# jiahuei/COMIC-Compact-Image-Captioning-with-Attention

Measured on AMD Instinct MI355X. Metric: images/sec (decoder-mode XE training, COMIC-256, InceptionV3 frozen), higher is better.
Workload: dtype bf16

## Files before the change

### comic-compact-image-captioning-with-attention_amd/_lib.py

```python
import ctypes as C
import os

_HERE = os.path.dirname(os.path.abspath(__file__))
LIB_PATH = os.environ.get('COMIC_HIP_LIB') or os.path.join(_HERE, 'lib', 'libcomic_hip.so')

c_void_p, c_int, c_int32, c_int64, c_float, c_double, c_char_p, c_uint64 = (
    C.c_void_p, C.c_int, C.c_int32, C.c_int64, C.c_float, C.c_double, C.c_char_p, C.c_uint64)


class CnnOp(C.Structure):
    _fields_ = [(n, c_int32) for n in (
        'kind', 'src', 'dst', 'src_coff', 'dst_coff', 'H', 'W', 'Cin', 'Cout', 'KH', 'KW', 'SH', 'SW',
        'PT', 'PL', 'Ho', 'Wo', 'weight', 'relu', 'out_f32', 'src_f32', 'lane', 'tile', 'group', 'flags', 'min_lds')]


class ImageDesc(C.Structure):
    _fields_ = [('offset', C.c_int64), ('in_h', c_int32), ('in_w', c_int32), ('flip', c_int32), ('oy', c_int32),
                ('ox', c_int32), ('sy', C.c_float), ('sx', C.c_float)]


class ConvWeight(C.Structure):
    _fields_ = [('w', c_void_p), ('scale', c_void_p), ('shift', c_void_p), ('w_frag', c_void_p)]


# ... 67 lines not shown
class BeamRequired(C.Structure):
    _fields_ = [('n_words', c_int32), ('stride', c_int32)]


class BeamSampling(C.Structure):
    _fields_ = [('temperature', c_float), ('seed_dev', c_void_p)]


class BeamTruncation(C.Structure):
    _fields_ = [('top_k', c_int32), ('top_p', c_float)]


class GemmProb(C.Structure):
    _fields_ = [(n, c_void_p) for n in ('A', 'B', 'C', 'bias', 'mask')] + [(n, c_int32) for n in (
        'M', 'N', 'K', 'lda', 'ldb', 'ldc', 'ld_mask')] + [(n, c_float) for n in ('alpha', 'beta', 'keep')] + [
        ('type', c_int32), ('ones_a', c_int32)]


class ConvGrad(C.Structure):
    _fields_ = [('w_master', c_void_p), ('dw', c_void_p), ('dbeta', c_void_p), ('w_bwd', c_void_p),
                ('bwd_tile', c_int32), ('reserved', c_int32)]


P = c_void_p
_SIGS = {
    'comic_last_error': (c_char_p, []),
    'comic_abi_version': (c_int, []),
    'comic_device_count': (c_int, []),
    'comic_pack_conv_weights': (c_int, [P, P, c_int, c_int, c_int, c_int, c_int, P]),
    'comic_fold_bn': (c_int, [P, P, P, c_float, P, P, c_int, P]),
    'comic_cnn_forward': (c_int, [P, c_int, P, P, P, c_int, c_int, P]),
    'comic_cnn_group_args_bytes': (C.c_long, [P, c_int]),
    'comic_cnn_build_group_args': (c_int, [P, c_int, P, P, P, c_int, P]),
    'comic_cnn_forward_grouped': (c_int, [P, c_int, P, P, P, c_int, c_int, P, P]),
    'comic_clip_by_norm': (c_int, [P, P, P, c_int, c_float, c_float, c_float, P, P, P]),
    'comic_cnn_backward_scratch_bytes': (c_int64, [P, c_int, c_int, c_int, c_int]),
    'comic_cnn_backward': (c_int, [P, c_int, P, P, P, P, P, c_int, c_int, c_int, P, c_int64, P, P]),
    'comic_cnn_backward_sched': (c_int, [P, c_int, P, c_int, P, P, P, P, P, P, c_int, c_int, c_int, P, c_int64, P, P, P]),
    'comic_cnn_pack_bwd_filters': (c_int, [P, c_int, P, c_int, P]),
    'comic_cnn_pack_x3_weights': (c_int, [P, P, P, P, P, c_int, P]),
    'comic_cnn_refresh_weights': (c_int, [P, P, c_int64, P, P, P, P, c_int64, P]),
    'comic_cnn_refresh_weights_dtype': (c_int, [P, P, c_int64, P, P, P, P, c_int64, c_int, P]),
    'comic_cnn_pack_frag_weights': (c_int, [P, P, P, c_int, c_int64, P]),
    'comic_crc32c': (C.c_uint32, [P, C.c_size_t, C.c_uint32]),
    'comic_conv2d_bn_relu': (c_int, [P, P, c_int, P, c_int, P, c_int, c_int, P]),
    'comic_gemm_f32': (c_int, [P, P, P, P, c_int, c_int, c_int, c_int, c_int, c_int, c_int, c_int, c_float,
                               c_float, P]),
    'comic_gemm_f32_split3': (c_int, [P, P, P, P, c_int, c_int, c_int, c_int, c_int, c_int, c_int, c_int, c_float,
                                      c_float, P, c_int64, P]),
    'comic_gemm_f32_splitk': (c_int, [P, P, P, P, c_int, c_int, c_int, c_int, c_int, c_int, c_int, c_int, c_float,
                                      c_float, P, c_int64, P]),
    'comic_gemm_group_workspace': (c_int64, [P, c_int]),
    'comic_gemm_group': (c_int, [P, c_int, P, c_int64, P]),
    'comic_embed_fwd': (c_int, [P, P, P, c_int, c_int, c_int, P]),
    'comic_embed_bwd': (c_int, [P, P, P, c_int, c_int, c_int, P]),
    'comic_dropout_apply': (c_int, [P, P, c_float, P, c_int64, P]),
    'comic_dropout_mask': (c_int, [P, c_int64, c_float, c_uint64, c_uint64, P]),
    'comic_dropout_mask_dev': (c_int, [P, c_int64, c_float, P, c_uint64, P]),
    'comic_dropout_masks4_dev': (c_int, [P, P, P, P, P]),
    'comic_image_preprocess': (c_int, [P, P, c_int, P, c_int, c_int, c_int, P]),
    'comic_jpeg_pixels': (c_int, [P, P, c_int, c_int, c_int, c_int, P, P, P]),
    'comic_jpeg_preprocess': (c_int, [P, P, c_int, c_int, P, P, P, P, c_int, c_int, c_int, P]),
    'comic_jpeg_preprocess_packed': (c_int, [P, P, c_int, c_int, P, P, P, P, c_int, c_int, c_int, P]),
    'comic_weighted_sum_tb': (c_int, [P, P, c_int, c_int, P, P]),
    'comic_lstm_gates_fwd': (c_int, [P, P, P, P, P, P, P, P, c_float, P, c_int, P, P, c_int, c_int, P]),
    'comic_lstm_gates_bwd': (c_int, [P, P, P, P, P, c_float, P, c_int, P, P, P, c_int, c_int, P]),
    'comic_attn_step_fwd': (c_int, [P, P, P, P, P, P, P, P, P, c_float, P, P, P, P]),
    'comic_attn_step_bwd': (c_int, [P, P, P, P, P, P, P, P, P, P, c_float, P, P, P, P, P, P, P]),
    'comic_xent_fwd_bwd': (c_int, [P, P, P, P, P, P, P, P, c_int, c_int, c_int, P]),
    'comic_argmax_rows': (c_int, [P, P, c_int, c_int, P]),
    'comic_beam_step': (c_int, [P, P, P, P, P, P, P, c_int, c_int, c_int, c_int, P]),
    'comic_gather_rows': (c_int, [P, P, P, c_int, c_int, c_int, P]),
    'comic_gather_tree': (c_int, [P, P, P, P, c_int, c_int, c_int, c_int, P]),
    'comic_adam_tf': (c_int, [P, P, P, P, c_int64, c_float, c_float, c_float, c_float, c_float, c_float, P]),
    'comic_adam_tf_gated': (c_int, [P, P, P, P, c_int64, c_float, c_float, c_float, c_float, c_float, c_float, P, P]),
    'comic_momentum_tf_gated': (c_int, [P, P, P, c_int64, c_float, c_float, c_float, c_float, P, P]),
    'comic_debug_occupy_cus': (c_int, [c_int, c_int, P]),
    'comic_colsum': (c_int, [P, P, c_int, c_int, c_float, P]),
    'comic_ln_tanh_fwd': (c_int, [P, P, P, P, P, c_int, c_int, c_float, P]),
    'comic_ln_tanh_bwd_rows': (c_int, [P, P, P, P, P, c_int, c_int, P]),
    'comic_momentum_tf': (c_int, [P, P, P, c_int64, c_float, c_float, c_float, c_float, P]),
    'comic_axpy': (c_int, [P, P, c_float, c_int64, P]),
    'comic_decoder_train_workspace': (c_int64, [P, c_int, c_int]),
    'comic_decoder_train_path': (c_int, []),
    'comic_decoder_greedy_path': (c_int, []),
    'comic_decoder_beam_path': (c_int, []),
    'comic_beam_step_dense_workspace': (c_int64, [c_int, c_int, c_int, c_int]),
    'comic_beam_step_dense': (c_int, [c_void_p] * 9 + [c_int] * 5 + [c_void_p, c_int64, c_void_p]),
    'comic_gemm_f32_stream_workspace': (c_int64, [c_int, c_int, c_int]),
    'comic_gemm_f32_stream': (c_int, [c_void_p, c_void_p, c_void_p, c_void_p, c_int, c_int, c_int, c_void_p, c_int64, c_void_p]),
    'comic_decoder_infer_workspace': (c_int64, [P, c_int, c_int]),
    'comic_decoder_train_step': (c_int, [P, P, P, P, P, P, P, P, P, P, c_int, c_int, c_int, P, P, P, P, P, P, P,
                                         P, P, P, P, P, c_int64, P]),
    'comic_decoder_score_workspace': (c_int64, [P, c_int, c_int]),
    'comic_decoder_score': (c_int, [P, P, P, P, P, P, P, P, c_int, c_int, c_int, P, P, P, P, c_int64, P]),
    'comic_decoder_score_path': (c_int, []),
    'comic_decoder_greedy': (c_int, [P, P, P, P, c_int, c_int, P, P, P, P, P, c_int64, P]),
    'comic_decoder_sample': (c_int, [P, P, P, P, c_int, c_int, P, P, P, P, P, P, c_int64, P]),
    'comic_decoder_beam': (c_int, [P, P, P, P, c_int, c_int, c_int, P, P, P, P, P, P, P, P, c_int64, P]),
    'comic_beam_step_ensemble_workspace': (c_int64, [c_int, c_int, c_int, c_int]),
    'comic_beam_step_ensemble': (c_int, [P, P, c_int, P, P, P, P, P, P, c_int, c_int, c_int, c_int, c_float, P, c_int64, P]),
    'comic_beam_step_ensemble_path': (c_int, []),
    'comic_decoder_beam_ensemble_workspace': (c_int64, [P, c_int, c_int, c_int]),
    'comic_decoder_beam_ensemble': (c_int, [P, P, P, P, P, c_int, c_int, c_int, c_int, P, P, P, P, P, P, P, P, c_int64, P]),
    'comic_beam_bans': (c_int, [P, P, P, P, P, P, c_int, c_int, c_int, c_int, c_int, c_int, P, P]),
    'comic_beam_step_constrained': (c_int, [P, P, c_int, P, P, P, P, P, P, c_int, c_int, c_int, c_int, c_float, P, c_int, P,
# ... 166 lines not shown
```

### comic-compact-image-captioning-with-attention_amd/csrc/gemm_group.h

```cpp
#pragma once
#include "common.h"

constexpr int kGemmGroupMax = 20;
enum { COMIC_GG_TN = 0, COMIC_GG_NN = 1, COMIC_GG_NT = 2 };

struct ComicGemmProb {
  const float* A;
  const float* B;
  float* C;
  const float* bias;
  const float* mask;
  int M, N, K, lda, ldb, ldc, ld_mask;
  float alpha, beta;
  float keep;
  int type;
  int ones_a;
  int tiles_m, tiles_n, S, k_per_slice, wg_begin;
  int slab_tile0;
  int ticket0;
};

struct ComicGemmGroup {
  ComicGemmProb p[kGemmGroupMax];
  int n;
  float* slab;
  unsigned* tickets;
  int xcd_chunk;
};

int comic_gemm_group_plan(ComicGemmGroup& g, int target_items, int64_t* slab_bytes, int* n_tickets);
constexpr int kGemmGroupTargetItems = 640;
int comic_gemm_group_launch(const ComicGemmGroup& g, int n_wg, hipStream_t st);
```

### comic-compact-image-captioning-with-attention_amd/csrc/gemm_group.hip

```cpp
#include <algorithm>

#include "gemm_group.h"
#include "gemm_x3_dev.h"

namespace {

constexpr int GB = 128;
constexpr int kGemmGroupSlots = 512;
constexpr int kItemOverhead = 6;
constexpr int kSc1 = 16;
typedef __attribute__((ext_vector_type(4))) unsigned gg_u32x4_t;

__device__ __forceinline__ __amdgpu_buffer_rsrc_t gg_rsrc(const void* p, long bytes) {
  return __builtin_amdgcn_make_buffer_rsrc((void*)p, 0, (int)bytes, 0x00020000);
}
__device__ __forceinline__ float4 gg_load16_sc1(__amdgpu_buffer_rsrc_t r, unsigned off) {
  const gg_u32x4_t v = __builtin_amdgcn_raw_buffer_load_b128(r, (int)off, 0, kSc1);
  return make_float4(__uint_as_float(v.x), __uint_as_float(v.y), __uint_as_float(v.z), __uint_as_float(v.w));
}
__device__ __forceinline__ void gg_store16_sc1(__amdgpu_buffer_rsrc_t r, unsigned off, float4 v) {
  const gg_u32x4_t u = {__float_as_uint(v.x), __float_as_uint(v.y), __float_as_uint(v.z), __float_as_uint(v.w)};
  __builtin_amdgcn_raw_buffer_store_b128(u, r, (int)off, 0, kSc1);
}

constexpr int kGroupLds = 4 * (X3Tile<GB, true>::BYTES + X3Tile<GB, true>::BYTES);
static_assert(X3Tile<GB, true>::BYTES >= X3Tile<GB, false>::BYTES, "LDS of the k-contiguous form bounds the others");
constexpr int kGroupLdsPc = 2 * 2 * (X3TilePc<GB, false>::BYTES + X3TilePc<GB, false>::BYTES);
static_assert(X3TilePc<GB, false>::BYTES >= X3TilePc<GB, true>::BYTES, "LDS of the row-contiguous form bounds the others");

__device__ __forceinline__ void gg_emit(const ComicGemmProb& p, int m, int n, float4 a) {
  if (m >= p.M || n >= p.N) return;
  const int nv = min(4, p.N - n);
  float v[4] = {a.x * p.alpha, a.y * p.alpha, a.z * p.alpha, a.w * p.alpha};
  float* cp = p.C + (size_t)m * p.ldc + n;
#pragma unroll
  for (int q = 0; q < 4; ++q) {
    if (q >= nv) break;
    if (p.bias) v[q] += p.bias[n + q];
    if (p.mask) v[q] = (v[q] / p.keep) * p.mask[(size_t)m * p.ld_mask + n + q];
    if (p.beta != 0.f) v[q] += p.beta * cp[q];
  }
  if (nv == 4 && (p.ldc % 4 == 0) && (((uintptr_t)p.C & 15) == 0)) {
    *(float4*)cp = make_float4(v[0], v[1], v[2], v[3]);
  } else {
#pragma unroll
    for (int q = 0; q < 4; ++q)
      if (q < nv) cp[q] = v[q];
  }
}

template <bool PC>
__global__ __launch_bounds__(PC ? 512 : 256) void gemm_group_x3_kernel(ComicGemmGroup g) {
  constexpr int NT = PC ? 512 : 256;
  constexpr int LDS = PC ? kGroupLdsPc : kGroupLds;
  extern __shared__ __attribute__((aligned(16))) unsigned char smem[];
  int bid = blockIdx.x;
  if (g.xcd_chunk > 0 && bid < g.xcd_chunk * 8) bid = (bid & 7) * g.xcd_chunk + (bid >> 3);
  volatile unsigned* s_last = (volatile unsigned*)(smem + LDS - 16);
  int pi = 0;
#pragma unroll 1
  for (int i = 1; i < g.n; ++i)
    if (bid >= g.p[i].wg_begin) pi = i;
  const ComicGemmProb& p = g.p[pi];
  const int local = bid - p.wg_begin;
  const int S = p.S, ntiles = p.tiles_m * p.tiles_n;
  const int slice = local / ntiles, tl = local - slice * ntiles;
  constexpr int PW = 8;
  const int panel = tl / (p.tiles_m * PW), rem = tl - panel * p.tiles_m * PW;
  const int pw = min(PW, p.tiles_n - panel * PW);
  const int mt = rem / pw, nt = panel * PW + rem % pw;
  const int tile = mt * p.tiles_n + nt;
  const int m0 = mt * GB, n0 = nt * GB;
  const int kbeg = S > 1 ? slice * p.k_per_slice : 0;
  const int kend = S > 1 ? min(p.K, kbeg + p.k_per_slice) : p.K;
  const int tid = threadIdx.x, lane = tid & 63, wave = tid >> 6;
  const int wm = wave >> 1, wn = wave & 1;

  const long tile_id = (long)p.ticket0 + tile;
  const __amdgpu_buffer_rsrc_t sr = gg_rsrc(g.slab + ((long)p.slab_tile0 + (long)tile * S) * (GB * GB), (long)S * GB * GB * 4);
  const unsigned sbase = (unsigned)slice * (GB * GB * 4);
  if (p.ones_a) {
    constexpr int KG = NT / 32;
    float4* red = (float4*)smem;
    const int cg = tid & 31, kg = tid >> 5, n = n0 + 4 * cg;
    const bool vec = (p.ldb % 4 == 0) && (((uintptr_t)p.B & 15) == 0);
    float4 sm = make_float4(0.f, 0.f, 0.f, 0.f);
    if (n < p.N)
      for (int k = kbeg + kg; k < kend; k += KG) {
        const float4 v = load4(p.B + (size_t)k * p.ldb + n, p.N - n, vec);
        sm.x += v.x; sm.y += v.y; sm.z += v.z; sm.w += v.w;
      }
    red[kg * 32 + cg] = sm;
    __syncthreads();
    if (tid < 32) {
      float4 tot = red[cg];
#pragma unroll
      for (int k = 1; k < KG; ++k) {
        const float4 v = red[k * 32 + cg];
        tot.x += v.x; tot.y += v.y; tot.z += v.z; tot.w += v.w;
      }
      if (S == 1) gg_emit(p, 0, n, tot);
      else gg_store16_sc1(sr, sbase + (unsigned)cg * 16u, tot);
    }
    if (S == 1) return;
  } else {
    f32x4_t acc[4][4];
    if constexpr (PC) {
      if (p.type == COMIC_GG_TN) x3_mainloop_pc<false, false>(p.A, p.B, p.M, p.N, p.lda, p.ldb, m0, n0, kbeg, kend, smem, acc);
      else if (p.type == COMIC_GG_NN) x3_mainloop_pc<true, false>(p.A, p.B, p.M, p.N, p.lda, p.ldb, m0, n0, kbeg, kend, smem, acc);
      else x3_mainloop_pc<true, true>(p.A, p.B, p.M, p.N, p.lda, p.ldb, m0, n0, kbeg, kend, smem, acc);
    } else {
      if (p.type == COMIC_GG_TN)
        x3_mainloop<GB, false, false, GB>(p.A, p.B, p.M, p.N, p.lda, p.ldb, m0, n0, kbeg, kend, smem, acc);
      else if (p.type == COMIC_GG_NN)
        x3_mainloop<GB, true, false, GB>(p.A, p.B, p.M, p.N, p.lda, p.ldb, m0, n0, kbeg, kend, smem, acc);
      else
        x3_mainloop<GB, true, true, GB>(p.A, p.B, p.M, p.N, p.lda, p.ldb, m0, n0, kbeg, kend, smem, acc);
    }
    const bool owner = wave < 4;
    if (S == 1) {
      if (owner)
#pragma unroll
      for (int i = 0; i < 4; ++i)
#pragma unroll
        for (int j = 0; j < 4; ++j)
          gg_emit(p, m0 + wm * 64 + j * 16 + (lane & 15), n0 + wn * 64 + i * 16 + (lane >> 4) * 4,
                  make_float4(acc[i][j][0], acc[i][j][1], acc[i][j][2], acc[i][j][3]));
      return;
    }
    if (owner)
#pragma unroll
    for (int i = 0; i < 4; ++i)
#pragma unroll
      for (int j = 0; j < 4; ++j) {
        const int ml = wm * 64 + j * 16 + (lane & 15), nl = wn * 64 + i * 16 + (lane >> 4) * 4;
        gg_store16_sc1(sr, sbase + (unsigned)(ml * GB + nl) * 4u, make_float4(acc[i][j][0], acc[i][j][1], acc[i][j][2], acc[i][j][3]));
      }
  }
  asm volatile("s_waitcnt vmcnt(0)" ::: "memory");
  __syncthreads();
  if (tid == 0) {
    const unsigned t = __hip_atomic_fetch_add(g.tickets + tile_id, 1u, __ATOMIC_RELAXED, __HIP_MEMORY_SCOPE_AGENT);
    *s_last = (t == (unsigned)(S - 1)) ? 1u : 0u;
    if (t == (unsigned)(S - 1)) __hip_atomic_store(g.tickets + tile_id, 0u, __ATOMIC_RELAXED, __HIP_MEMORY_SCOPE_AGENT);
  }
  __syncthreads();
  if (!*s_last) return;
  const int n_chunks = p.ones_a ? 1 : (GB * GB / 4) / NT;
#pragma unroll 1
  for (int c = 0; c < n_chunks; c += 4) {
    float4 sum[4];
#pragma unroll
    for (int u = 0; u < 4; ++u) sum[u] = make_float4(0.f, 0.f, 0.f, 0.f);
#pragma unroll 1
    for (int s = 0; s < S; ++s) {
      float4 v[4];
#pragma unroll
      for (int u = 0; u < 4; ++u) v[u] = gg_load16_sc1(sr, (unsigned)s * (GB * GB * 4) + (unsigned)(tid + NT * (c + u)) * 16u);
#pragma unroll
      for (int u = 0; u < 4; ++u) {
        sum[u].x += v[u].x; sum[u].y += v[u].y; sum[u].z += v[u].z; sum[u].w += v[u].w;
      }
    }
// ... 16 lines not shown
    COMIC_REQUIRE(p.M > 0 && p.N > 0 && p.K > 0 && p.B && p.C && (p.A || p.ones_a), "gemm_group: bad problem %d", i);
    COMIC_REQUIRE(p.type >= COMIC_GG_TN && p.type <= COMIC_GG_NT, "gemm_group: bad type of problem %d", i);
    COMIC_REQUIRE(!p.ones_a || (p.type == COMIC_GG_TN && p.M == 1), "gemm_group: ones_a needs type TN and M = 1 (problem %d)", i);
    COMIC_REQUIRE(p.ldc >= p.N && (!p.mask || p.ld_mask >= p.N), "gemm_group: leading dimension of problem %d", i);
    if (!p.ones_a) COMIC_REQUIRE(p.lda >= (p.type == COMIC_GG_TN ? p.M : p.K), "gemm_group: lda of problem %d", i);
    COMIC_REQUIRE(p.ldb >= (p.type == COMIC_GG_NT ? p.K : p.N), "gemm_group: ldb of problem %d", i);
    p.tiles_m = cdiv(p.M, GB);
    p.tiles_n = cdiv(p.N, GB);
    cost += (long)cdiv(p.M, GB) * p.tiles_n * cdiv(p.K, 32);
  }
  auto split_of = [](int kt, long klen) { return (int)std::min<long>(16, std::max<long>(1, (kt + klen / 2) / klen)); };
  long klen = std::max<long>(8, cost / std::max(1, target_items));
  {
    long best = -1, best_klen = klen, kt_max = 8;
    for (int i = 0; i < g.n; ++i) kt_max = std::max<long>(kt_max, cdiv(g.p[i].K, 32));
    for (long kl = klen; kl <= kt_max; ++kl) {
      long items = 0, longest = 0;
      for (int i = 0; i < g.n; ++i) {
        const ComicGemmProb& p = g.p[i];
        const int kt = cdiv(p.K, 32), S = split_of(kt, kl);
        items += (long)p.tiles_m * p.tiles_n * S;
        if (!p.ones_a) longest = std::max<long>(longest, cdiv(kt, S));
      }
      const long est = cdiv64(items, kGemmGroupSlots) * (longest + kItemOverhead);
      if (best < 0 || est < best) {
        best = est;
        best_klen = kl;
      }
    }
    klen = best_klen;
  }
  int wg = 0, tickets = 0, slab_tiles = 0;
  for (int i = 0; i < g.n; ++i) {
    ComicGemmProb& p = g.p[i];
    const int nt = cdiv(p.M, GB) * p.tiles_n, kt = cdiv(p.K, 32);
    int S = split_of(kt, klen);
    p.k_per_slice = cdiv(kt, S) * 32;
    S = cdiv(p.K, p.k_per_slice);
    p.S = S;
    p.wg_begin = wg;
    p.slab_tile0 = slab_tiles;
    p.ticket0 = tickets;
    wg += nt * S;
    if (S > 1) {
      slab_tiles += nt * S;
      tickets += nt;
    }
  }
  if (slab_bytes) *slab_bytes = (int64_t)slab_tiles * GB * GB * 4;
  if (n_tickets) *n_tickets = tickets;
  return wg;
}

int comic_gemm_group_launch(const ComicGemmGroup& g_in, int n_wg, hipStream_t st) {
  ComicGemmGroup g = g_in;
  g.xcd_chunk = n_wg / 8;
  COMIC_REQUIRE(n_wg > 0, "gemm_group: empty launch");
  bool pc = n_wg <= 256;
  for (int i = 0; i < g.n && pc; ++i) {
    const ComicGemmProb& p = g.p[i];
    if (p.ones_a) continue;
    const bool a_kc = p.type != COMIC_GG_TN, b_kc = p.type == COMIC_GG_NT;
    pc = p.lda % 4 == 0 && p.ldb % 4 == 0 && ((uintptr_t)p.A & 15) == 0 && ((uintptr_t)p.B & 15) == 0 &&
         (!(a_kc || b_kc) || p.K % 4 == 0);
  }
  static PerDeviceOnce once, once_pc;
  bool& done = pc ? once_pc.slot() : once.slot();
  const int lds = pc ? kGroupLdsPc : kGroupLds;
  if (!done) {
    const void* fn = pc ? (const void*)gemm_group_x3_kernel<true> : (const void*)gemm_group_x3_kernel<false>;
    COMIC_REQUIRE(hipFuncSetAttribute(fn, hipFuncAttributeMaxDynamicSharedMemorySize, lds) == hipSuccess,
                  "gemm_group: cannot reserve %d bytes of LDS", lds);
    done = true;
  }
  if (pc) hipLaunchKernelGGL(gemm_group_x3_kernel<true>, dim3((unsigned)n_wg), dim3(512), lds, st, g);
  else hipLaunchKernelGGL(gemm_group_x3_kernel<false>, dim3((unsigned)n_wg), dim3(256), lds, st, g);
  COMIC_LAUNCH_CHECK("gemm_group");
  return 0;
}

namespace {
int gg_from_public(const comic_gemm_prob* probs, int n, ComicGemmGroup& g) {
  COMIC_REQUIRE(probs && n > 0 && n <= kGemmGroupMax, "gemm_group: 1..%d problems", kGemmGroupMax);
  g = ComicGemmGroup{};
  g.n = n;
  for (int i = 0; i < n; ++i) {
    const comic_gemm_prob& q = probs[i];
    ComicGemmProb& p = g.p[i];
    p.A = q.A; p.B = q.B; p.C = q.C; p.bias = q.bias; p.mask = q.mask;
    p.M = q.M; p.N = q.N; p.K = q.K; p.lda = q.lda; p.ldb = q.ldb; p.ldc = q.ldc; p.ld_mask = q.ld_mask;
    p.alpha = q.alpha; p.beta = q.beta; p.keep = q.keep; p.type = q.type; p.ones_a = q.ones_a;
  }
  return 0;
}
#define kPublicTarget kGemmGroupTargetItems
}

extern "C" int64_t comic_gemm_group_workspace(const comic_gemm_prob* probs, int n) {
  ComicGemmGroup g;
  if (gg_from_public(probs, n, g)) return -1;
  int64_t slab = 0;
  int nt = 0;
  if (comic_gemm_group_plan(g, kPublicTarget, &slab, &nt) < 0) return -1;
  return slab + 256 + (int64_t)nt * 4;
}

extern "C" int comic_gemm_group(const comic_gemm_prob* probs, int n, void* workspace, int64_t workspace_bytes, void* stream) {
  ComicGemmGroup g;
  if (int rc = gg_from_public(probs, n, g)) return rc;
  int64_t slab = 0;
  int nt = 0;
  const int wg = comic_gemm_group_plan(g, kPublicTarget, &slab, &nt);
  if (wg < 0) return 2;
  const int64_t slab_al = (slab + 255) / 256 * 256;
  COMIC_REQUIRE(nt == 0 || (workspace && workspace_bytes >= slab_al + (int64_t)nt * 4), "gemm_group: workspace too small");
  g.slab = (float*)workspace;
  g.tickets = nt ? (unsigned*)((char*)workspace + slab_al) : nullptr;
  if (nt) COMIC_REQUIRE(hipMemsetAsync(g.tickets, 0, (size_t)nt * 4, (hipStream_t)stream) == hipSuccess, "gemm_group: memset");
  return comic_gemm_group_launch(g, wg, (hipStream_t)stream);
}
```

### comic-compact-image-captioning-with-attention_amd/csrc/gemm_x3_dev.h

```cpp
#pragma once
#include <type_traits>

#include "common.h"

namespace {

__device__ __forceinline__ float4 load4(const float* __restrict__ p, int nvalid, bool vec_ok) {
  if (nvalid >= 4 && vec_ok) return *(const float4*)p;
  float4 r = make_float4(0.f, 0.f, 0.f, 0.f);
  if (nvalid > 0) r.x = p[0];
  if (nvalid > 1) r.y = p[1];
  if (nvalid > 2) r.z = p[2];
  if (nvalid > 3) r.w = p[3];
  return r;
}

__device__ __forceinline__ void split_bf16x2(float a, float b, uint32_t& hi, uint32_t& lo) {
  hi = pack_bf16x2(a, b);
  lo = pack_bf16x2(a - __uint_as_float(hi << 16), b - __uint_as_float(hi & 0xFFFF0000u));
}

template <int ROWS, bool KC>
struct X3Tile {
  static constexpr int ROWB = 80;
// ... 205 lines not shown
    }
#pragma unroll
    for (int j = 0; j < TM; ++j) {
      ah[j] = x3_frag<BM, A_KC>(Ah + P * ABYTES, wm * (BM / 2) + j * 16, lane);
      al[j] = x3_frag<BM, A_KC>(Al + P * ABYTES, wm * (BM / 2) + j * 16, lane);
    }
#pragma unroll
    for (int i = 0; i < TN; ++i)
#pragma unroll
      for (int j = 0; j < TM; ++j) {
        acc[i][j] = __builtin_amdgcn_mfma_f32_16x16x32_bf16(bl[i], ah[j], acc[i][j], 0, 0, 0);
        acc[i][j] = __builtin_amdgcn_mfma_f32_16x16x32_bf16(bh[i], al[j], acc[i][j], 0, 0, 0);
        acc[i][j] = __builtin_amdgcn_mfma_f32_16x16x32_bf16(bh[i], ah[j], acc[i][j], 0, 0, 0);
      }
    sa.mask(kbeg + (kt + 1) * BKx, tid, ar[P ^ 1]);
    sb.mask(kbeg + (kt + 1) * BKx, tid, br[P ^ 1]);
    x3_store_tile<BM, A_KC, ACH>(Ah + (P ^ 1) * ABYTES, Al + (P ^ 1) * ABYTES, tid, ar[P ^ 1]);
    x3_store_tile<BN, B_KC, BCH>(Bh + (P ^ 1) * BBYTES, Bl + (P ^ 1) * BBYTES, tid, br[P ^ 1]);
#ifdef COMIC_X3_SCHED
    __builtin_amdgcn_sched_group_barrier(0x020, ACH + BCH, 0);
    __builtin_amdgcn_sched_group_barrier(0x100, 64, 0);
#pragma unroll
    for (int r = 0; r < TM * TN; ++r) {
      __builtin_amdgcn_sched_group_barrier(0x008, 3, 0);
      __builtin_amdgcn_sched_group_barrier(0x002, 9, 0);
      __builtin_amdgcn_sched_group_barrier(0x200, 1, 0);
    }
#endif
    __syncthreads();
  };
  for (int kt = 0; kt < nk; kt += 2) {
    step(kt, std::integral_constant<int, 0>());
    step(kt + 1, std::integral_constant<int, 1>());
  }
}

template <int BM, bool A_KC, bool B_KC, int BN>
__device__ __forceinline__ void x3_mainloop(const float* __restrict__ A, const float* __restrict__ B, int M, int N, int lda,
                                            int ldb, int m0, int n0, int kbeg, int kend, unsigned char* smem,
                                            f32x4_t (&acc)[BN / 32][BM / 32]) {
  const bool a_vec = (lda % 4 == 0) && (((uintptr_t)A & 15) == 0) && (!A_KC || kend % 4 == 0);
  const bool b_vec = (ldb % 4 == 0) && (((uintptr_t)B & 15) == 0) && (!B_KC || kend % 4 == 0);
  if (a_vec && b_vec) x3_mainloop_v<BM, A_KC, B_KC, BN, true>(A, B, M, N, lda, ldb, m0, n0, kbeg, kend, smem, acc);
  else x3_mainloop_v<BM, A_KC, B_KC, BN, false>(A, B, M, N, lda, ldb, m0, n0, kbeg, kend, smem, acc);
}

template <int ROWS, bool KC>
struct X3TilePc {
  static constexpr int KSTR = 2 * ROWS + 32;
  static constexpr int BYTES = KC ? ROWS * 64 : 32 * KSTR;
};
__device__ __forceinline__ int x3_swz(int row) { return (0x6C >> (((row >> 2) & 3) * 2)) & 3; }

template <int ROWS, bool KC, int NCH>
__device__ __forceinline__ void x3pc_store_tile(unsigned char* hi_base, unsigned char* lo_base, int tid,
                                                const float4 (&in)[NCH]) {
  using T = X3TilePc<ROWS, KC>;
#pragma unroll
  for (int i = 0; i < NCH; ++i) {
    const int q = tid + 256 * i;
    uint32_t h0, l0, h1, l1;
    split_bf16x2(in[i].x, in[i].y, h0, l0);
    split_bf16x2(in[i].z, in[i].w, h1, l1);
    int off;
    if (KC) {
      const int row = q >> 3, c = q & 7;
      off = row * 64 + (((c & 3) ^ x3_swz(row)) * 2 + (c >> 2)) * 8;
    } else {
      constexpr int CPR = ROWS / 4;
      const int kk = q / CPR, row = (q % CPR) * 4;
      off = kk * T::KSTR + row * 2;
    }
    *(uint2*)(hi_base + off) = make_uint2(h0, h1);
    *(uint2*)(lo_base + off) = make_uint2(l0, l1);
  }
}
template <int ROWS, bool KC>
__device__ __forceinline__ bf16x8_t x3pc_frag(const unsigned char* base, int row16, int lane) {
  using T = X3TilePc<ROWS, KC>;
  if (KC) {
    const int row = row16 + (lane & 15);
    const uint4 v = *(const uint4*)(base + row * 64 + (((lane >> 4) ^ x3_swz(row)) * 16));
    return __builtin_bit_cast(bf16x8_t, v);
  } else {
    const int g = lane >> 4, q = (lane >> 2) & 3, pp = lane & 3;
    const unsigned char* p = base + (4 * g + q) * T::KSTR + (row16 + 4 * pp) * 2;
    const uint32_t a0 = (uint32_t)(uintptr_t)((__attribute__((address_space(3))) const unsigned char*)p);
    const x3_s16x4_t lo = __builtin_amdgcn_ds_read_tr16_b64_v4i16((__attribute__((address_space(3))) x3_s16x4_t*)(uintptr_t)a0);
    const x3_s16x4_t hi =
        __builtin_amdgcn_ds_read_tr16_b64_v4i16((__attribute__((address_space(3))) x3_s16x4_t*)(uintptr_t)(a0 + 16 * T::KSTR));
    const x3_s16x8_t v = {lo[0], lo[1], lo[2], lo[3], hi[0], hi[1], hi[2], hi[3]};
    return __builtin_bit_cast(bf16x8_t, v);
  }
}

template <bool A_KC, bool B_KC>
__device__ __forceinline__ void x3_mainloop_pc(const float* __restrict__ A, const float* __restrict__ B, int M, int N, int lda,
                                               int ldb, int m0, int n0, int kbeg, int kend, unsigned char* smem,
                                               f32x4_t (&acc)[4][4]) {
  constexpr int BM = 128, BN = 128, BKx = 32, NCH = 4;
  constexpr int ABYTES = X3TilePc<BM, A_KC>::BYTES, BBYTES = X3TilePc<BN, B_KC>::BYTES;
  constexpr int STAGE = 2 * (ABYTES + BBYTES);
  const int tid = threadIdx.x, lane = tid & 63;
  const int wave = __builtin_amdgcn_readfirstlane(tid >> 6);
  const int nk = ((kend - kbeg + BKx - 1) / BKx + 3) & ~3;
#pragma unroll
  for (int i = 0; i < 4; ++i)
#pragma unroll
    for (int j = 0; j < 4; ++j) acc[i][j] = (f32x4_t){0.f, 0.f, 0.f, 0.f};
  if (wave >= 4) {
    const int pt = tid - 256;
    X3Src<BM, A_KC, NCH, true> sa;
    X3Src<BN, B_KC, NCH, true> sb;
    sa.init(A, lda, m0, M, kbeg, kend, pt);
    sb.init(B, ldb, n0, N, kbeg, kend, pt);
    float4 ar[4][NCH], br[4][NCH];
#pragma unroll
    for (int s = 0; s < 4; ++s) {
      sa.load(kbeg + s * BKx, pt, ar[s]);
      sb.load(kbeg + s * BKx, pt, br[s]);
    }
    auto put = [&](int stage, const float4 (&a)[NCH], const float4 (&b)[NCH]) {
      unsigned char* st = smem + stage * STAGE;
      x3pc_store_tile<BM, A_KC, NCH>(st, st + ABYTES, pt, a);
      x3pc_store_tile<BN, B_KC, NCH>(st + 2 * ABYTES, st + 2 * ABYTES + BBYTES, pt, b);
    };
    put(0, ar[0], br[0]);
    sa.load(kbeg + 4 * BKx, pt, ar[0]);
    sb.load(kbeg + 4 * BKx, pt, br[0]);
    __syncthreads();
    auto step = [&](int kt, auto s_) {
      constexpr int S = decltype(s_)::value;
      put(S & 1, ar[S], br[S]);
      sa.load(kbeg + (kt + 5) * BKx, pt, ar[S]);
      sb.load(kbeg + (kt + 5) * BKx, pt, br[S]);
      __syncthreads();
    };
    for (int kt = 0; kt < nk; kt += 4) {
      step(kt, std::integral_constant<int, 1>());
      step(kt + 1, std::integral_constant<int, 2>());
      step(kt + 2, std::integral_constant<int, 3>());
      step(kt + 3, std::integral_constant<int, 0>());
    }
  } else {
    const int wm = wave >> 1, wn = wave & 1;
    __syncthreads();
    auto step = [&](auto p_) {
      constexpr int P = decltype(p_)::value;
      const unsigned char* st = smem + P * STAGE;
      bf16x8_t bh[4], bl[4], ah[4], al[4];
#pragma unroll
      for (int i = 0; i < 4; ++i) {
        bh[i] = x3pc_frag<BN, B_KC>(st + 2 * ABYTES, wn * 64 + i * 16, lane);
        bl[i] = x3pc_frag<BN, B_KC>(st + 2 * ABYTES + BBYTES, wn * 64 + i * 16, lane);
      }
#pragma unroll
      for (int j = 0; j < 4; ++j) {
        ah[j] = x3pc_frag<BM, A_KC>(st, wm * 64 + j * 16, lane);
        al[j] = x3pc_frag<BM, A_KC>(st + ABYTES, wm * 64 + j * 16, lane);
      }
#pragma unroll
      for (int i = 0; i < 4; ++i)
#pragma unroll
        for (int j = 0; j < 4; ++j) {
          acc[i][j] = __builtin_amdgcn_mfma_f32_16x16x32_bf16(bl[i], ah[j], acc[i][j], 0, 0, 0);
          acc[i][j] = __builtin_amdgcn_mfma_f32_16x16x32_bf16(bh[i], al[j], acc[i][j], 0, 0, 0);
          acc[i][j] = __builtin_amdgcn_mfma_f32_16x16x32_bf16(bh[i], ah[j], acc[i][j], 0, 0, 0);
        }
      __syncthreads();
    };
    for (int kt = 0; kt < nk; kt += 2) {
      step(std::integral_constant<int, 0>());
      step(std::integral_constant<int, 1>());
    }
  }
}

}
```

### include/comic_hip.h

```cpp
#ifndef COMIC_HIP_H_
#define COMIC_HIP_H_

#include <stddef.h>
#include <stdint.h>

#ifdef __cplusplus
extern "C" {
#endif

#define COMIC_F32 0
#define COMIC_BF16 1
#define COMIC_F16 2
#define COMIC_ABI_VERSION 1
#define COMIC_CONV_TILES 61
#define COMIC_WS_TILE 54
#define COMIC_IMG_TILE 55
#define COMIC_CHAIN_TILE 62

const char* comic_last_error(void);
int comic_abi_version(void);
int comic_device_count(void);


int comic_pack_conv_weights(const float* w_hwio, void* w_packed, int kh, int kw, int cin, int cout,
// ... 69 lines not shown
  float* dbeta;
  void* w_bwd;
  int32_t bwd_tile;
  int32_t reserved;
} comic_conv_grad;
int64_t comic_cnn_backward_scratch_bytes(const comic_cnn_op* ops, int n_ops, int batch, int dtype, int lanes);
int comic_cnn_backward(const comic_cnn_op* ops, int n_ops, void* const* buffers,
                       void* const* grad_buffers, const int32_t* buf_channels,
                       const comic_conv_weight* weights, const comic_conv_grad* grads, int batch,
                       int dtype, int filters_ready ,
                       void* scratch, int64_t scratch_bytes, void* stream, void* wgrad_stream);
#define COMIC_CNN_BWD_NO_ACT_FUSION 2
int comic_cnn_backward_sched(const comic_cnn_op* ops, int n_ops, const int32_t* sched, int n_sched, void* const* buffers,
                             void* const* grad_buffers, void* const* grad_buffers_alt, const int32_t* buf_channels,
                             const comic_conv_weight* weights, const comic_conv_grad* grads, int batch, int dtype,
                             int filters_ready, void* scratch, int64_t scratch_bytes, void* stream0, void* stream1,
                             void* wgrad_stream);
int comic_cnn_pack_x3_weights(const float* const* masters, void* const* outs, const int32_t* cout, const int32_t* taps,
                              const int32_t* cin, int n, void* stream);
int comic_cnn_pack_bwd_filters(const comic_cnn_op* ops, int n_ops, const comic_conv_grad* grads,
                               int dtype, void* stream);
int comic_cnn_refresh_weights(const float* master, void* plan_copy, int64_t n, const float* beta,
                              const float* mean, const float* scale, float* shift,
                              int64_t channels, void* stream);
int comic_cnn_refresh_weights_dtype(const float* master, void* plan_copy, int64_t n, const float* beta,
                                    const float* mean, const float* scale, float* shift,
                                    int64_t channels, int dtype, void* stream);

int comic_conv2d_bn_relu(const comic_cnn_op* op, const void* x, int x_channels, void* y,
                         int y_channels, const comic_conv_weight* wt, int batch, int dtype,
                         void* stream);

int comic_gemm_f32(const float* A, const float* B, float* C, const float* bias, int M, int N, int K,
                   int lda, int ldb, int ldc, int trans_a, int trans_b, float alpha, float beta,
                   void* stream);

int comic_gemm_f32_split3(const float* A, const float* B, float* C, const float* bias, int M, int N,
                          int K, int lda, int ldb, int ldc, int trans_a, int trans_b, float alpha,
                          float beta, void* workspace ,
                          int64_t workspace_bytes, void* stream);

typedef struct comic_gemm_prob {
  const float* A;
  const float* B;
  float* C;
  const float* bias;
  const float* mask;
  int32_t M, N, K, lda, ldb, ldc, ld_mask;
  float alpha, beta, keep;
  int32_t type, ones_a;
} comic_gemm_prob;
int64_t comic_gemm_group_workspace(const comic_gemm_prob* probs, int n);
int comic_gemm_group(const comic_gemm_prob* probs, int n, void* workspace, int64_t workspace_bytes, void* stream);

int64_t comic_gemm_f32_stream_workspace(int R, int Kin, int N);
int comic_gemm_f32_stream(const float* x, const float* W, const float* bias, float* out, int R, int Kin, int N,
                          void* workspace, int64_t workspace_bytes, void* stream);

int comic_gemm_f32_splitk(const float* A, const float* B, float* C, const float* bias, int M, int N,
                          int K, int lda, int ldb, int ldc, int trans_a, int trans_b, float alpha,
                          float beta, void* workspace, int64_t workspace_bytes, void* stream);

int comic_embed_fwd(const float* table, const int32_t* ids, float* out, int rows, int E, int V,
                    void* stream);
int comic_embed_bwd(const int32_t* ids, const float* dout, float* dtable, int rows, int E, int V,
                    void* stream);

int comic_dropout_apply(const float* x, const float* mask, float keep, float* y, int64_t n,
                        void* stream);
int comic_dropout_mask(float* mask, int64_t n, float keep, uint64_t seed, uint64_t offset,
                       void* stream);
int comic_dropout_mask_dev(float* mask, int64_t n, float keep, const uint64_t* seed_dev,
                           uint64_t offset, void* stream);
int comic_dropout_masks4_dev(float* mask, const int64_t* n4, const float* keep4, const uint64_t* seed_dev,
                             void* stream);
int comic_weighted_sum_tb(const float* rows_tb, const float* w_bt, int T, int B, float* out, void* stream);

int comic_lstm_gates_fwd(const float* g, const float* c_prev, const float* h_prev, float* gates_act,
                         float* c_new, float* h_new, float* y, const float* mask_out, float keep_out,
                         const int32_t* lens, int t, float* c_state, float* h_state, int B, int D,
                         void* stream);
int comic_lstm_gates_bwd(const float* gates_act, const float* c_prev, const float* c_new,
                         const float* dy, const float* mask_out, float keep_out, const int32_t* lens,
                         int t, float* dc_state, float* dh_state, float* dg, int B, int D, void* stream);

typedef struct comic_attn_desc {
  int32_t B, M, D, H, Cv;
  int32_t method;
  int32_t prob;
  int32_t tied;
} comic_attn_desc;

int comic_attn_step_fwd(const comic_attn_desc* d, const float* keys, const float* values,
                        const float* q, const float* ln_g, const float* ln_b, const float* v,
                        const float* tau, const float* mask_alpha, float keep_alpha, float* alpha,
                        float* alpha_d, float* ctx, void* stream);
int comic_attn_step_bwd(const comic_attn_desc* d, const float* keys, const float* values,
                        const float* q, const float* ln_g, const float* ln_b, const float* v,
                        const float* tau, const float* alpha, const float* mask_alpha,
                        float keep_alpha, const float* dctx, const float* dmap, float* dq,
                        float* dkeys, float* dvalues, float* pgrad, void* stream);

int comic_xent_fwd_bwd(float* logits, const int32_t* targets_bt, const float* coef_bt,
                       const float* wmask_bt, const int32_t* lens, float* loss_rows, float* dlogits,
                       int32_t* ids_tb, int T, int B, int V, void* stream);

// ... 308 lines not shown
```

Before: 39590.

## Add a register-lean producer/consumer grouped-GEMM form and make it the default

Adds a third grouped-GEMM kernel form that uses producer/consumer waves with a prefetch depth of 2 instead of 4, double-buffered B fragments, and sched barriers. It requests 4 waves per EU so more workgroups can be resident. The default now picks this form whenever operands allow 16-byte loads, dropping the old limit of at most 256 workgroups. The shallower prefetch risks exposing more global-load latency, and the change also adds an explicit form-selection entry point and an occupancy query.

```diff
diff --git a/comic-compact-image-captioning-with-attention_amd/_lib.py b/comic-compact-image-captioning-with-attention_amd/_lib.py
--- a/comic-compact-image-captioning-with-attention_amd/_lib.py
+++ b/comic-compact-image-captioning-with-attention_amd/_lib.py
@@ -143,6 +143,8 @@
                                       c_float, P, c_int64, P]),
     'comic_gemm_group_workspace': (c_int64, [P, c_int]),
     'comic_gemm_group': (c_int, [P, c_int, P, c_int64, P]),
+    'comic_gemm_group_form': (c_int, [P, c_int, P, c_int64, c_int, P]),
+    'comic_gemm_group_resident': (c_int, [c_int]),
     'comic_embed_fwd': (c_int, [P, P, P, c_int, c_int, c_int, P]),
     'comic_embed_bwd': (c_int, [P, P, P, c_int, c_int, c_int, P]),
     'comic_dropout_apply': (c_int, [P, P, c_float, P, c_int64, P]),
diff --git a/comic-compact-image-captioning-with-attention_amd/csrc/gemm_group.h b/comic-compact-image-captioning-with-attention_amd/csrc/gemm_group.h
--- a/comic-compact-image-captioning-with-attention_amd/csrc/gemm_group.h
+++ b/comic-compact-image-captioning-with-attention_amd/csrc/gemm_group.h
@@ -30,4 +30,4 @@
 
 int comic_gemm_group_plan(ComicGemmGroup& g, int target_items, int64_t* slab_bytes, int* n_tickets);
 constexpr int kGemmGroupTargetItems = 640;
-int comic_gemm_group_launch(const ComicGemmGroup& g, int n_wg, hipStream_t st);
+int comic_gemm_group_launch(const ComicGemmGroup& g, int n_wg, hipStream_t st, int form = 0);
diff --git a/comic-compact-image-captioning-with-attention_amd/csrc/gemm_group.hip b/comic-compact-image-captioning-with-attention_amd/csrc/gemm_group.hip
--- a/comic-compact-image-captioning-with-attention_amd/csrc/gemm_group.hip
+++ b/comic-compact-image-captioning-with-attention_amd/csrc/gemm_group.hip
@@ -49,8 +49,13 @@
   }
 }
 
-template <bool PC>
-__global__ __launch_bounds__(PC ? 512 : 256) void gemm_group_x3_kernel(ComicGemmGroup g) {
+template <int FORM>
+__global__ __launch_bounds__(FORM == 1 ? 256 : 512)
+#if defined(__HIP_DEVICE_COMPILE__)
+__attribute__((amdgpu_waves_per_eu(FORM == 3 ? 4 : 1, FORM == 3 ? 4 : 2)))
+#endif
+void gemm_group_x3_kernel(ComicGemmGroup g) {
+  constexpr bool PC = FORM != 1;
   constexpr int NT = PC ? 512 : 256;
   constexpr int LDS = PC ? kGroupLdsPc : kGroupLds;
   extern __shared__ __attribute__((aligned(16))) unsigned char smem[];
@@ -80,17 +85,17 @@
   const __amdgpu_buffer_rsrc_t sr = gg_rsrc(g.slab + ((long)p.slab_tile0 + (long)tile * S) * (GB * GB), (long)S * GB * GB * 4);
   const unsigned sbase = (unsigned)slice * (GB * GB * 4);
   if (p.ones_a) {
-    constexpr int KG = NT / 32;
+    constexpr int KG = 8;
     float4* red = (float4*)smem;
     const int cg = tid & 31, kg = tid >> 5, n = n0 + 4 * cg;
     const bool vec = (p.ldb % 4 == 0) && (((uintptr_t)p.B & 15) == 0);
     float4 sm = make_float4(0.f, 0.f, 0.f, 0.f);
-    if (n < p.N)
+    if (n < p.N && kg < KG)
       for (int k = kbeg + kg; k < kend; k += KG) {
         const float4 v = load4(p.B + (size_t)k * p.ldb + n, p.N - n, vec);
         sm.x += v.x; sm.y += v.y; sm.z += v.z; sm.w += v.w;
       }
-    red[kg * 32 + cg] = sm;
+    if (kg < KG) red[kg * 32 + cg] = sm;
     __syncthreads();
     if (tid < 32) {
       float4 tot = red[cg];
@@ -106,9 +111,10 @@
   } else {
     f32x4_t acc[4][4];
     if constexpr (PC) {
-      if (p.type == COMIC_GG_TN) x3_mainloop_pc<false, false>(p.A, p.B, p.M, p.N, p.lda, p.ldb, m0, n0, kbeg, kend, smem, acc);
-      else if (p.type == COMIC_GG_NN) x3_mainloop_pc<true, false>(p.A, p.B, p.M, p.N, p.lda, p.ldb, m0, n0, kbeg, kend, smem, acc);
-      else x3_mainloop_pc<true, true>(p.A, p.B, p.M, p.N, p.lda, p.ldb, m0, n0, kbeg, kend, smem, acc);
+      constexpr int DEPTH = FORM == 3 ? 2 : 4;
+      if (p.type == COMIC_GG_TN) x3_mainloop_pc<false, false, DEPTH>(p.A, p.B, p.M, p.N, p.lda, p.ldb, m0, n0, kbeg, kend, smem, acc);
+      else if (p.type == COMIC_GG_NN) x3_mainloop_pc<true, false, DEPTH>(p.A, p.B, p.M, p.N, p.lda, p.ldb, m0, n0, kbeg, kend, smem, acc);
+      else x3_mainloop_pc<true, true, DEPTH>(p.A, p.B, p.M, p.N, p.lda, p.ldb, m0, n0, kbeg, kend, smem, acc);
     } else {
       if (p.type == COMIC_GG_TN)
         x3_mainloop<GB, false, false, GB>(p.A, p.B, p.M, p.N, p.lda, p.ldb, m0, n0, kbeg, kend, smem, acc);
@@ -231,29 +237,46 @@
   return wg;
 }
 
-int comic_gemm_group_launch(const ComicGemmGroup& g_in, int n_wg, hipStream_t st) {
+namespace {
+bool gg_vec_ok(const ComicGemmGroup& g) {
+  for (int i = 0; i < g.n; ++i) {
+    const ComicGemmProb& p = g.p[i];
+    if (p.ones_a) continue;
+    const bool a_kc = p.type != COMIC_GG_TN, b_kc = p.type == COMIC_GG_NT;
+    if (!(p.lda % 4 == 0 && p.ldb % 4 == 0 && ((uintptr_t)p.A & 15) == 0 && ((uintptr_t)p.B & 15) == 0 &&
+          (!(a_kc || b_kc) || p.K % 4 == 0)))
+      return false;
+  }
+  return true;
+}
+const void* gg_kernel(int form) {
+  return form == 1 ? (const void*)gemm_group_x3_kernel<1> : form == 2 ? (const void*)gemm_group_x3_kernel<2> : (const void*)gemm_group_x3_kernel<3>;
+}
+int gg_lds(int form) { return form == 1 ? kGroupLds : kGroupLdsPc; }
+int gg_reserve_lds(int form) {
+  static PerDeviceOnce once[3];
+  bool& done = once[form - 1].slot();
+  if (!done) {
+    COMIC_REQUIRE(hipFuncSetAttribute(gg_kernel(form), hipFuncAttributeMaxDynamicSharedMemorySize, gg_lds(form)) == hipSuccess,
+                  "gemm_group: cannot reserve %d bytes of LDS", gg_lds(form));
+    done = true;
+  }
+  return 0;
+}
+}
+
+int comic_gemm_group_launch(const ComicGemmGroup& g_in, int n_wg, hipStream_t st, int form) {
   ComicGemmGroup g = g_in;
   g.xcd_chunk = n_wg / 8;
   COMIC_REQUIRE(n_wg > 0, "gemm_group: empty launch");
-  bool pc = n_wg <= 256;
-  for (int i = 0; i < g.n && pc; ++i) {
-    const ComicGemmProb& p = g.p[i];
-    if (p.ones_a) continue;
-    const bool a_kc = p.type != COMIC_GG_TN, b_kc = p.type == COMIC_GG_NT;
-    pc = p.lda % 4 == 0 && p.ldb % 4 == 0 && ((uintptr_t)p.A & 15) == 0 && ((uintptr_t)p.B & 15) == 0 &&
-         (!(a_kc || b_kc) || p.K % 4 == 0);
-  }
-  static PerDeviceOnce once, once_pc;
-  bool& done = pc ? once_pc.slot() : once.slot();
-  const int lds = pc ? kGroupLdsPc : kGroupLds;
-  if (!done) {
-    const void* fn = pc ? (const void*)gemm_group_x3_kernel<true> : (const void*)gemm_group_x3_kernel<false>;
-    COMIC_REQUIRE(hipFuncSetAttribute(fn, hipFuncAttributeMaxDynamicSharedMemorySize, lds) == hipSuccess,
-                  "gemm_group: cannot reserve %d bytes of LDS", lds);
-    done = true;
-  }
-  if (pc) hipLaunchKernelGGL(gemm_group_x3_kernel<true>, dim3((unsigned)n_wg), dim3(512), lds, st, g);
-  else hipLaunchKernelGGL(gemm_group_x3_kernel<false>, dim3((unsigned)n_wg), dim3(256), lds, st, g);
+  COMIC_REQUIRE(form >= 0 && form <= 3, "gemm_group: form %d", form);
+  const bool vec = gg_vec_ok(g);
+  if (form == 0) form = vec ? 3 : 1;
+  COMIC_REQUIRE(form == 1 || vec, "gemm_group: form %d needs 16-byte loadable operands", form);
+  if (int rc = gg_reserve_lds(form)) return rc;
+  if (form == 1) hipLaunchKernelGGL(gemm_group_x3_kernel<1>, dim3((unsigned)n_wg), dim3(256), kGroupLds, st, g);
+  else if (form == 2) hipLaunchKernelGGL(gemm_group_x3_kernel<2>, dim3((unsigned)n_wg), dim3(512), kGroupLdsPc, st, g);
+  else hipLaunchKernelGGL(gemm_group_x3_kernel<3>, dim3((unsigned)n_wg), dim3(512), kGroupLdsPc, st, g);
   COMIC_LAUNCH_CHECK("gemm_group");
   return 0;
 }
@@ -284,17 +307,38 @@
   return slab + 256 + (int64_t)nt * 4;
 }
 
-extern "C" int comic_gemm_group(const comic_gemm_prob* probs, int n, void* workspace, int64_t workspace_bytes, void* stream) {
+extern "C" int comic_gemm_group_form(const comic_gemm_prob* probs, int n, void* workspace, int64_t workspace_bytes, int form,
+                                     void* stream) {
+  COMIC_REQUIRE(form >= 0 && form <= 3, "gemm_group: form %d", form);
   ComicGemmGroup g;
   if (int rc = gg_from_public(probs, n, g)) return rc;
   int64_t slab = 0;
   int nt = 0;
   const int wg = comic_gemm_group_plan(g, kPublicTarget, &slab, &nt);
   if (wg < 0) return 2;
+  COMIC_REQUIRE(form < 2 || gg_vec_ok(g), "gemm_group: form %d needs 16-byte loadable operands", form);
   const int64_t slab_al = (slab + 255) / 256 * 256;
   COMIC_REQUIRE(nt == 0 || (workspace && workspace_bytes >= slab_al + (int64_t)nt * 4), "gemm_group: workspace too small");
   g.slab = (float*)workspace;
   g.tickets = nt ? (unsigned*)((char*)workspace + slab_al) : nullptr;
   if (nt) COMIC_REQUIRE(hipMemsetAsync(g.tickets, 0, (size_t)nt * 4, (hipStream_t)stream) == hipSuccess, "gemm_group: memset");
-  return comic_gemm_group_launch(g, wg, (hipStream_t)stream);
-}
+  return comic_gemm_group_launch(g, wg, (hipStream_t)stream, form);
+}
+
+extern "C" int comic_gemm_group(const comic_gemm_prob* probs, int n, void* workspace, int64_t workspace_bytes, void* stream) {
+  return comic_gemm_group_form(probs, n, workspace, workspace_bytes, 0, stream);
+}
+
+extern "C" int comic_gemm_group_resident(int form) {
+  if (form < 1 || form > 3) {
+    comic_set_error("gemm_group: form %d", form);
+    return -1;
+  }
+  if (gg_reserve_lds(form)) return -1;
+  int nb = 0;
+  if (hipOccupancyMaxActiveBlocksPerMultiprocessor(&nb, gg_kernel(form), form == 1 ? 256 : 512, gg_lds(form)) != hipSuccess) {
+    comic_set_error("gemm_group: occupancy query failed");
+    return -1;
+  }
+  return nb;
+}
diff --git a/comic-compact-image-captioning-with-attention_amd/csrc/gemm_x3_dev.h b/comic-compact-image-captioning-with-attention_amd/csrc/gemm_x3_dev.h
--- a/comic-compact-image-captioning-with-attention_amd/csrc/gemm_x3_dev.h
+++ b/comic-compact-image-captioning-with-attention_amd/csrc/gemm_x3_dev.h
@@ -281,12 +281,13 @@
 };
 __device__ __forceinline__ int x3_swz(int row) { return (0x6C >> (((row >> 2) & 3) * 2)) & 3; }
 
-template <int ROWS, bool KC, int NCH>
+template <int ROWS, bool KC, int NCH, bool TIGHT = false>
 __device__ __forceinline__ void x3pc_store_tile(unsigned char* hi_base, unsigned char* lo_base, int tid,
                                                 const float4 (&in)[NCH]) {
   using T = X3TilePc<ROWS, KC>;
 #pragma unroll
   for (int i = 0; i < NCH; ++i) {
+    if (TIGHT) __builtin_amdgcn_sched_barrier(0);
     const int q = tid + 256 * i;
     uint32_t h0, l0, h1, l1;
     split_bf16x2(in[i].x, in[i].y, h0, l0);
@@ -323,79 +324,107 @@
   }
 }
 
-template <bool A_KC, bool B_KC>
+template <bool A_KC, bool B_KC, int DEPTH>
 __device__ __forceinline__ void x3_mainloop_pc(const float* __restrict__ A, const float* __restrict__ B, int M, int N, int lda,
                                                int ldb, int m0, int n0, int kbeg, int kend, unsigned char* smem,
                                                f32x4_t (&acc)[4][4]) {
+  static_assert(DEPTH == 2 || DEPTH == 4, "register sets of the producers");
   constexpr int BM = 128, BN = 128, BKx = 32, NCH = 4;
   constexpr int ABYTES = X3TilePc<BM, A_KC>::BYTES, BBYTES = X3TilePc<BN, B_KC>::BYTES;
   constexpr int STAGE = 2 * (ABYTES + BBYTES);
   const int tid = threadIdx.x, lane = tid & 63;
   const int wave = __builtin_amdgcn_readfirstlane(tid >> 6);
-  const int nk = ((kend - kbeg + BKx - 1) / BKx + 3) & ~3;
-#pragma unroll
-  for (int i = 0; i < 4; ++i)
-#pragma unroll
-    for (int j = 0; j < 4; ++j) acc[i][j] = (f32x4_t){0.f, 0.f, 0.f, 0.f};
+  const int nk = ((kend - kbeg + BKx - 1) / BKx + DEPTH - 1) & ~(DEPTH - 1);
   if (wave >= 4) {
     const int pt = tid - 256;
     X3Src<BM, A_KC, NCH, true> sa;
     X3Src<BN, B_KC, NCH, true> sb;
     sa.init(A, lda, m0, M, kbeg, kend, pt);
     sb.init(B, ldb, n0, N, kbeg, kend, pt);
-    float4 ar[4][NCH], br[4][NCH];
-#pragma unroll
-    for (int s = 0; s < 4; ++s) {
+    float4 ar[DEPTH][NCH], br[DEPTH][NCH];
+#pragma unroll
+    for (int s = 0; s < DEPTH; ++s) {
       sa.load(kbeg + s * BKx, pt, ar[s]);
       sb.load(kbeg + s * BKx, pt, br[s]);
     }
     auto put = [&](int stage, const float4 (&a)[NCH], const float4 (&b)[NCH]) {
       unsigned char* st = smem + stage * STAGE;
-      x3pc_store_tile<BM, A_KC, NCH>(st, st + ABYTES, pt, a);
-      x3pc_store_tile<BN, B_KC, NCH>(st + 2 * ABYTES, st + 2 * ABYTES + BBYTES, pt, b);
+      x3pc_store_tile<BM, A_KC, NCH, DEPTH == 2>(st, st + ABYTES, pt, a);
+      x3pc_store_tile<BN, B_KC, NCH, DEPTH == 2>(st + 2 * ABYTES, st + 2 * ABYTES + BBYTES, pt, b);
+      if (DEPTH == 2) __builtin_amdgcn_sched_barrier(0);
     };
     put(0, ar[0], br[0]);
-    sa.load(kbeg + 4 * BKx, pt, ar[0]);
-    sb.load(kbeg + 4 * BKx, pt, br[0]);
+    sa.load(kbeg + DEPTH * BKx, pt, ar[0]);
+    sb.load(kbeg + DEPTH * BKx, pt, br[0]);
     __syncthreads();
     auto step = [&](int kt, auto s_) {
       constexpr int S = decltype(s_)::value;
       put(S & 1, ar[S], br[S]);
-      sa.load(kbeg + (kt + 5) * BKx, pt, ar[S]);
-      sb.load(kbeg + (kt + 5) * BKx, pt, br[S]);
+      sa.load(kbeg + (kt + 1 + DEPTH) * BKx, pt, ar[S]);
+      sb.load(kbeg + (kt + 1 + DEPTH) * BKx, pt, br[S]);
       __syncthreads();
     };
-    for (int kt = 0; kt < nk; kt += 4) {
-      step(kt, std::integral_constant<int, 1>());
-      step(kt + 1, std::integral_constant<int, 2>());
-      step(kt + 2, std::integral_constant<int, 3>());
-      step(kt + 3, std::integral_constant<int, 0>());
+    for (int kt = 0; kt < nk; kt += DEPTH) {
+      if constexpr (DEPTH == 4) {
+        step(kt, std::integral_constant<int, 1>());
+        step(kt + 1, std::integral_constant<int, 2>());
+        step(kt + 2, std::integral_constant<int, 3>());
+        step(kt + 3, std::integral_constant<int, 0>());
+      } else {
+        step(kt, std::integral_constant<int, 1>());
+        step(kt + 1, std::integral_constant<int, 0>());
+      }
     }
   } else {
     const int wm = wave >> 1, wn = wave & 1;
+#pragma unroll
+    for (int i = 0; i < 4; ++i)
+#pragma unroll
+      for (int j = 0; j < 4; ++j) acc[i][j] = (f32x4_t){0.f, 0.f, 0.f, 0.f};
     __syncthreads();
     auto step = [&](auto p_) {
       constexpr int P = decltype(p_)::value;
       const unsigned char* st = smem + P * STAGE;
-      bf16x8_t bh[4], bl[4], ah[4], al[4];
-#pragma unroll
-      for (int i = 0; i < 4; ++i) {
-        bh[i] = x3pc_frag<BN, B_KC>(st + 2 * ABYTES, wn * 64 + i * 16, lane);
-        bl[i] = x3pc_frag<BN, B_KC>(st + 2 * ABYTES + BBYTES, wn * 64 + i * 16, lane);
-      }
+      bf16x8_t ah[4], al[4];
 #pragma unroll
       for (int j = 0; j < 4; ++j) {
         ah[j] = x3pc_frag<BM, A_KC>(st, wm * 64 + j * 16, lane);
         al[j] = x3pc_frag<BM, A_KC>(st + ABYTES, wm * 64 + j * 16, lane);
       }
-#pragma unroll
-      for (int i = 0; i < 4; ++i)
-#pragma unroll
-        for (int j = 0; j < 4; ++j) {
-          acc[i][j] = __builtin_amdgcn_mfma_f32_16x16x32_bf16(bl[i], ah[j], acc[i][j], 0, 0, 0);
-          acc[i][j] = __builtin_amdgcn_mfma_f32_16x16x32_bf16(bh[i], al[j], acc[i][j], 0, 0, 0);
-          acc[i][j] = __builtin_amdgcn_mfma_f32_16x16x32_bf16(bh[i], ah[j], acc[i][j], 0, 0, 0);
-        }
+      if constexpr (DEPTH == 4) {
+        bf16x8_t bh[4], bl[4];
+#pragma unroll
+        for (int i = 0; i < 4; ++i) {
+          bh[i] = x3pc_frag<BN, B_KC>(st + 2 * ABYTES, wn * 64 + i * 16, lane);
+          bl[i] = x3pc_frag<BN, B_KC>(st + 2 * ABYTES + BBYTES, wn * 64 + i * 16, lane);
+        }
+#pragma unroll
+        for (int i = 0; i < 4; ++i)
+#pragma unroll
+          for (int j = 0; j < 4; ++j) {
+            acc[i][j] = __builtin_amdgcn_mfma_f32_16x16x32_bf16(bl[i], ah[j], acc[i][j], 0, 0, 0);
+            acc[i][j] = __builtin_amdgcn_mfma_f32_16x16x32_bf16(bh[i], al[j], acc[i][j], 0, 0, 0);
+            acc[i][j] = __builtin_amdgcn_mfma_f32_16x16x32_bf16(bh[i], ah[j], acc[i][j], 0, 0, 0);
+          }
+      } else {
+        bf16x8_t bh[2], bl[2];
+        bh[0] = x3pc_frag<BN, B_KC>(st + 2 * ABYTES, wn * 64, lane);
+        bl[0] = x3pc_frag<BN, B_KC>(st + 2 * ABYTES + BBYTES, wn * 64, lane);
+#pragma unroll
+        for (int i = 0; i < 4; ++i) {
+          if (i < 3) {
+            bh[(i + 1) & 1] = x3pc_frag<BN, B_KC>(st + 2 * ABYTES, wn * 64 + (i + 1) * 16, lane);
+            bl[(i + 1) & 1] = x3pc_frag<BN, B_KC>(st + 2 * ABYTES + BBYTES, wn * 64 + (i + 1) * 16, lane);
+          }
+#pragma unroll
+          for (int j = 0; j < 4; ++j) {
+            acc[i][j] = __builtin_amdgcn_mfma_f32_16x16x32_bf16(bl[i & 1], ah[j], acc[i][j], 0, 0, 0);
+            acc[i][j] = __builtin_amdgcn_mfma_f32_16x16x32_bf16(bh[i & 1], al[j], acc[i][j], 0, 0, 0);
+            acc[i][j] = __builtin_amdgcn_mfma_f32_16x16x32_bf16(bh[i & 1], ah[j], acc[i][j], 0, 0, 0);
+          }
+          __builtin_amdgcn_sched_barrier(0);
+        }
+      }
       __syncthreads();
     };
     for (int kt = 0; kt < nk; kt += 2) {
diff --git a/include/comic_hip.h b/include/comic_hip.h
--- a/include/comic_hip.h
+++ b/include/comic_hip.h
@@ -145,6 +145,9 @@
 } comic_gemm_prob;
 int64_t comic_gemm_group_workspace(const comic_gemm_prob* probs, int n);
 int comic_gemm_group(const comic_gemm_prob* probs, int n, void* workspace, int64_t workspace_bytes, void* stream);
+int comic_gemm_group_form(const comic_gemm_prob* probs, int n, void* workspace, int64_t workspace_bytes, int form,
+                          void* stream);
+int comic_gemm_group_resident(int form);
 
 int64_t comic_gemm_f32_stream_workspace(int R, int Kin, int N);
 int comic_gemm_f32_stream(const float* x, const float* W, const float* bias, float* out, int R, int Kin, int N,
```

Result: faster. 40080, median of 6 (+1.2%).
